# fchchen/omni-recall-rag

Measured on AMD Instinct MI355X. Metric: queries/sec at top-k=10 over N x 3072-d chunks; score delta vs C# reference in `parity`, higher is better.
Workload: dtype i8 screen + f32*f32->f64 exact re-score; 1 GPU; C3: 10000000 chunks x 3072-d fp32 on one GPU, batch=256 queries per step, top-k=10, full hybrid (cosine+keyword+recency), candidate_limit=corpus; corpus_rows=10000000

## Files before the change

include/omnirecall_hip.h:

```cpp
#ifndef OMNIRECALL_HIP_H
#define OMNIRECALL_HIP_H

#include <stddef.h>
#include <stdint.h>

#ifdef __cplusplus
extern "C" {
#endif

#define ORR_ABI_VERSION 1

typedef enum orr_status {
    ORR_OK      = 0,
    ORR_EINVAL  = -1,
    ORR_ENOMEM  = -2,
    ORR_EDEVICE = -3,
    ORR_ECOMM   = -4,
    ORR_EDIM    = -5,
    ORR_ESTATE  = -6
} orr_status;

typedef struct orr_index orr_index;

typedef struct orr_config {
// ... 160 lines not shown
                              int64_t now_ticks, int32_t topk, int64_t candidate_limit, const orr_scope *scope,
                              int64_t *out_rows, double *out_scores, int32_t *out_counts);

int orr_search_batch_in_scopes(orr_index *idx, int32_t B, int32_t dim, const float *q,
                               const uint8_t *terms_utf8, const uint32_t *term_off, const uint32_t *query_term_off,
                               int64_t now_ticks, int32_t topk, int64_t candidate_limit,
                               int32_t n_scopes, const orr_scope *const *scopes, const int32_t *query_scope ,
                               int64_t *out_rows, double *out_scores, int32_t *out_counts);

int orr_index_set_option(orr_index *idx, const char *name, int64_t value);

int orr_index_screen_dots(orr_index *idx, int32_t B, int32_t dim, const float *q, float *out);

int orr_index_screen_i8_dots(orr_index *idx, int32_t B, int32_t dim, const float *q, int32_t form, int32_t nt_rows,
                             int32_t *out_dots, int8_t *out_iq, int8_t *out_ie);

int orr_index_screen_i8_consts(orr_index *idx, int32_t B, int32_t dim, const float *q, float *out_scale, float *out_rel_err,
                               float *out_rel_hat, float *out_rowf, float *out_s1, double *out_err2, double *out_err2_level1,
                               int8_t *out_iq2);

int orr_index_screen_i8_stream_dots(orr_index *idx, int32_t B, int32_t dim, const float *q, int32_t unit16, int32_t *out_dots);

int orr_index_pass_dots(orr_index *idx, int32_t kernel, int32_t B, int32_t dim, const float *q, float *out);

int orr_index_set_profiling(orr_index *idx, int32_t enabled);
int orr_index_kernel_stats(orr_index *idx, orr_kernel_stat *out, int32_t cap);

int orr_index_search_stats(orr_index *idx, orr_search_stats *out, int32_t reset);

typedef struct orr_cluster orr_cluster;
int        orr_cluster_create(const int32_t *devices, int32_t n_shards, int32_t dim, int64_t capacity_rows_per_shard,
                              orr_cluster **out);
void       orr_cluster_destroy(orr_cluster *c);
int32_t    orr_cluster_shards(const orr_cluster *c);
orr_index *orr_cluster_shard(orr_cluster *c, int32_t i);
int        orr_cluster_seal(orr_cluster *c);
int64_t    orr_cluster_rows(const orr_cluster *c);
int        orr_cluster_search_batch(orr_cluster *c, int32_t B, int32_t dim, const float *q_host,
                                    const uint8_t *terms_utf8, const uint32_t *term_off,
                                    const uint32_t *query_term_off, int64_t now_ticks, int32_t topk,
                                    int64_t candidate_limit, int64_t *out_rows, double *out_scores,
                                    int32_t *out_counts);
int        orr_cluster_search_batch_scoped(orr_cluster *c, int32_t B, int32_t dim, const float *q_host,
                                           const uint8_t *terms_utf8, const uint32_t *term_off,
                                           const uint32_t *query_term_off, int64_t now_ticks, int32_t topk,
                                           int64_t candidate_limit, int64_t n_scope_ids, const int64_t *scope_ids,
// ... 20 lines not shown
```

omni-recall-rag_amd/_native.py:

```python
from __future__ import annotations

import ctypes as C
import os

_PKG = os.path.dirname(os.path.abspath(__file__))
HIP_LIB_PATH = os.environ.get("ORR_HIP_LIB") or os.path.join(_PKG, "libomnirecall_hip.so")
HOST_LIB_PATH = os.path.join(_PKG, "libomnirecall_host.so")


class OrrError(RuntimeError):
    def __init__(self, code: int, message: str):
        super().__init__(f"libomnirecall_hip status {code}: {message}")
        self.code = code


ORR_OK, ORR_EINVAL, ORR_ENOMEM, ORR_EDEVICE, ORR_ECOMM, ORR_EDIM, ORR_ESTATE = 0, -1, -2, -3, -4, -5, -6
ORR_CAND_TRAILER, ORR_CAND_DOT_EXACT, ORR_CAND_DEAD = 1, 2, 16
ORR_SCOPE_AND, ORR_SCOPE_OR, ORR_SCOPE_ANDNOT = 0, 1, 2


class OrrConfig(C.Structure):
    _fields_ = [("struct_size", C.c_int32), ("device", C.c_int32), ("dim", C.c_int32), ("flags", C.c_int32),
                ("capacity_rows", C.c_int64), ("row_base", C.c_int64)]

# ... 96 lines not shown
hip.orr_index_update_rows.argtypes = [_vp, _i64, _vp, _i32, _vp, _vp]
hip.orr_index_insert_rows.restype = C.c_int
hip.orr_index_insert_rows.argtypes = [_vp, _i64, _i32, _vp, _vp, _vp, _vp, _vp, _vp]
hip.orr_cluster_insert_rows.restype = C.c_int
hip.orr_cluster_insert_rows.argtypes = [_vp, _i32, _i64, _i32, _vp, _vp, _vp, _vp, _vp, _vp]
hip.orr_index_compact.restype = C.c_int
hip.orr_index_compact.argtypes = [_vp, _vp]
hip.orr_cluster_compact.restype = C.c_int
hip.orr_cluster_compact.argtypes = [_vp, _vp]
hip.orr_index_live_rows.restype = _i64
hip.orr_index_live_rows.argtypes = [_vp]
hip.orr_index_view.restype = C.c_int
hip.orr_index_view.argtypes = [_vp, C.POINTER(_vp)]
hip.orr_index_screen_dots.restype = C.c_int
hip.orr_index_screen_dots.argtypes = [_vp, _i32, _i32, _vp, _vp]
hip.orr_index_screen_i8_dots.restype = C.c_int
hip.orr_index_screen_i8_dots.argtypes = [_vp, _i32, _i32, _vp, _i32, _i32, _vp, _vp, _vp]
hip.orr_index_screen_i8_consts.restype = C.c_int
hip.orr_index_screen_i8_consts.argtypes = [_vp, _i32, _i32, _vp, _vp, _vp, _vp, _vp, _vp, _vp, _vp, _vp]
hip.orr_index_screen_i8_stream_dots.restype = C.c_int
hip.orr_index_screen_i8_stream_dots.argtypes = [_vp, _i32, _i32, _vp, _i32, _vp]
hip.orr_index_pass_dots.restype = C.c_int
hip.orr_index_pass_dots.argtypes = [_vp, _i32, _i32, _i32, _vp, _vp]
hip.orr_index_set_profiling.restype = C.c_int
hip.orr_index_set_profiling.argtypes = [_vp, _i32]
hip.orr_index_kernel_stats.restype = C.c_int
hip.orr_index_kernel_stats.argtypes = [_vp, _vp, _i32]
hip.orr_index_search_stats.restype = C.c_int
hip.orr_index_search_stats.argtypes = [_vp, C.POINTER(OrrSearchStats), _i32]
hip.orr_cluster_create.restype = C.c_int
hip.orr_cluster_create.argtypes = [_vp, _i32, _i32, _i64, C.POINTER(_vp)]
hip.orr_cluster_destroy.restype = None
hip.orr_cluster_destroy.argtypes = [_vp]
hip.orr_cluster_shards.restype = _i32
hip.orr_cluster_shards.argtypes = [_vp]
hip.orr_cluster_shard.restype = _vp
hip.orr_cluster_shard.argtypes = [_vp, _i32]
hip.orr_cluster_seal.restype = C.c_int
hip.orr_cluster_seal.argtypes = [_vp]
hip.orr_cluster_rows.restype = _i64
hip.orr_cluster_rows.argtypes = [_vp]
hip.orr_cluster_search_batch.restype = C.c_int
hip.orr_cluster_search_batch.argtypes = [_vp, _i32, _i32, _vp, _vp, _vp, _vp, _i64, _i32, _i64, _vp, _vp, _vp]
hip.orr_cluster_search_batch_scoped.restype = C.c_int
hip.orr_cluster_search_batch_scoped.argtypes = [_vp, _i32, _i32, _vp, _vp, _vp, _vp, _i64, _i32, _i64, _i64, _vp, _vp, _vp, _vp, _vp]
hip.orr_cluster_search_batch_masked.restype = C.c_int
# ... 61 lines not shown
host.orrh_batcher_create.restype = _vp
host.orrh_batcher_create.argtypes = [_vp, _i32, _i32]
host.orrh_batcher_destroy.restype = None
host.orrh_batcher_destroy.argtypes = [_vp]
host.orrh_batcher_search.restype = C.c_int
host.orrh_batcher_search.argtypes = [_vp, _i32, _vp, _vp, _vp, _i32, _i64, _i32, _i64, _vp, _vp, _vp]
host.orrh_batcher_search_at.restype = C.c_int
host.orrh_batcher_search_at.argtypes = [_vp, _i32, _vp, _vp, _vp, _i32, _i64, _i32, _i64, _vp, _vp, _vp, _vp]
host.orrh_batcher_stats.restype = None
host.orrh_batcher_stats.argtypes = [_vp, _vp, _vp, _vp]
host.orrh_batcher_create.restype = _vp
host.orrh_batcher_create.argtypes = [_vp, _i32, _i32]
host.orrh_batcher_destroy.restype = None
host.orrh_batcher_destroy.argtypes = [_vp]
host.orrh_batcher_search.restype = C.c_int
host.orrh_batcher_search.argtypes = [_vp, _i32, _vp, _vp, _vp, _i32, _i64, _i32, _i64, _vp, _vp, _vp]
host.orrh_batcher_stats.restype = None
host.orrh_batcher_stats.argtypes = [_vp, _vp, _vp, _vp]

EXPORTED_HIP_SYMBOLS = [
    "orr_abi_version", "orr_device_count", "orr_last_error", "orr_index_create", "orr_index_destroy",
    "orr_index_append", "orr_index_seal", "orr_index_rows", "orr_index_dim", "orr_search_batch",
    "orr_search_shard", "orr_search_shard_ex", "orr_search_batch_scoped", "orr_search_batch_masked", "orr_search_batch_masked_groups", "orr_search_shard_scoped", "orr_search_shard_masked", "orr_index_scope_count", "orr_merge_candidates", "orr_merge_candidates_ex", "orr_index_set_profiling", "orr_index_kernel_stats",
    "orr_index_save", "orr_index_load", "orr_index_set_row_base", "orr_index_set_option", "orr_index_screen_dots", "orr_index_screen_i8_dots", "orr_index_screen_i8_consts", "orr_index_screen_i8_stream_dots", "orr_index_pass_dots", "orr_index_view",
    "orr_index_delete_rows", "orr_index_update_rows", "orr_index_insert_rows", "orr_cluster_insert_rows", "orr_index_live_rows", "orr_index_compact", "orr_cluster_compact", "orr_index_search_stats",
    "orr_cluster_create", "orr_cluster_destroy", "orr_cluster_shards", "orr_cluster_shard", "orr_cluster_seal", "orr_cluster_rows",
    "orr_cluster_search_batch", "orr_cluster_search_batch_scoped", "orr_cluster_search_batch_masked", "orr_cluster_search_stats", "orr_cluster_set_option",
    "orr_scope_create", "orr_scope_create_ticks", "orr_scope_add_ids", "orr_scope_combine", "orr_scope_rows", "orr_scope_row_ids", "orr_scope_destroy",
    "orr_search_batch_in_scope", "orr_search_batch_in_scopes",
]
EXPORTED_HOST_SYMBOLS = ["orrh_is_blank", "orrh_lower_invariant", "orrh_query_terms", "orrh_build_snippet",
                         "orrh_round4", "orrh_has_sufficient_evidence", "orrh_format_score_f4", "orrh_last_error", "orrh_store_create", "orrh_store_destroy",
                         "orrh_store_upsert_document", "orrh_store_upsert_chunks", "orrh_store_delete_document",
                         "orrh_store_chunk_count", "orrh_store_import_cosmos_json", "orrh_store_export_cosmos_json", "orrh_service_create", "orrh_service_destroy",
                         "orrh_service_search_json", "orrh_service_search_documents_json", "orrh_service_stats", "orrh_service_tombstoned_rows", "orrh_service_compactions", "orrh_service_delta_merges", "orrh_service_updated_rows", "orrh_service_inserted_rows", "orrh_service_set_option", "orrh_free", "orrh_batcher_create", "orrh_batcher_destroy",
                         "orrh_batcher_search", "orrh_batcher_search_at", "orrh_batcher_stats"]


def check(status: int) -> None:
    if status != ORR_OK:
        raise OrrError(status, (hip.orr_last_error() or b"").decode("utf-8", "replace"))
```

omni-recall-rag_amd/csrc/orr_api.hip:

```cpp
#include <hip/hip_runtime.h>

#include <algorithm>
#include <cmath>
#include <cstdarg>
#include <cstdio>
#include <chrono>
#include <pthread.h>
#include <dlfcn.h>
#include <atomic>
#include <condition_variable>
#include <functional>
#include <cstring>
#include <limits>
#include <mutex>
#include <shared_mutex>
#include <deque>
#include <new>
#include <numeric>
#include <string>
#include <string_view>
#include <thread>
#include <unordered_map>
#include <vector>

// ... 3209 lines not shown
                HIP_TRY(orr::launch_fuse_select(io.d_dot, io.d_dotf, n, idx->d_norm_b, idx->d_created, io.d_rowc, io.kw, qc, a.now_ticks,
                                                n, B, 0, sample_seg, nullptr, idx->ws_sel.as<orr::SelEntry>(), 0, s));
            }
            Timed t(idx, "select_floor", 0.0);
            HIP_TRY(orr::launch_select_final_sample(idx->ws_sel.as<orr::SelEntry>(), n_seg32, sample_seg, B, kprime, d_tau, s));
        }
        {
            Timed t(idx, "fuse_select", (double)B * (double)n * (8.0 * (p.use_cos ? 1 : 0) + 8.0 + 8.0));
            HIP_TRY(orr::launch_fuse_select(io.d_dot, io.d_dotf, n, idx->d_norm_b, idx->d_created, io.d_rowc, io.kw, qc, a.now_ticks,
                                            n, B, sample_seg, n_seg32 - sample_seg, d_tau, idx->ws_sel.as<orr::SelEntry>(), 0, s));
        }
        Timed t(idx, "select_final", (double)B * (double)n_seg * orr::kSelWidth * sizeof(orr::SelEntry));
        HIP_TRY(orr::launch_select_final(idx->ws_sel.as<orr::SelEntry>(), n_seg32, B, kprime, n, idx->row_base,
                                         io.d_dot, io.d_dotf, n, idx->d_norm_b, idx->d_created, idx->d_row_ids, io.kw,
                                         p.use_mfma ? 0 : 1, p.approx_eps, nullptr, nullptr, 0u, nullptr, io.d_cand, s));
    }
    if (p.use_mfma && !p.two_stage()) {
        Timed t(idx, "rescore_exact", (double)B * kprime * 4.0 * idx->dim);
        HIP_TRY(orr::launch_rescore_exact(idx->d_emb, idx->dim, io.d_q, B, kprime, idx->row_base, io.d_cand, s));
    }
    return ORR_OK;
}

int finish_pass(orr_index *idx, const BatchArgs &a, const PassPlan &p, const KwSide &kws, uint32_t n_terms_total)
{
    const int32_t B = a.B;
    HIP_TRY(hipStreamSynchronize(idx->stream));
    if (kws.bm_bytes) {
        if (kws.bm_bytes >= ((size_t)16 << 20)) {
            HIP_TRY(hipMemsetAsync(idx->ws_bitmaps.p, 0, kws.bm_bytes, idx->stream_aux));
            HIP_TRY(hipEventRecord(idx->ev_bm_clean, idx->stream_aux));
            idx->bm_clean_pending = true;
        } else {
            HIP_TRY(hipMemsetAsync(idx->ws_bitmaps.p, 0, kws.bm_bytes, idx->stream_kw));
        }
        idx->bitmaps_clean = std::max(kws.bm_bytes, kws.bm_clean_before);
    }
    if (n_terms_total > 0 && idx->ws_counter.p) {
        HIP_TRY(hipMemsetAsync(idx->ws_counter.p, 0, sizeof(unsigned long long), idx->stream_kw));
        if (idx->ws_kwalias.p) HIP_TRY(hipMemsetAsync(idx->ws_kwalias.p, 0, idx->ws_kwalias.cap, idx->stream_kw));
        idx->kw_counters_clean = true;
        idx->kw_counters_of[0] = idx->ws_counter.p;
        idx->kw_counters_of[1] = idx->ws_kwalias.p;
    }
    if (p.dev_norms) memcpy(idx->h_norm_a.data(), idx->pin_norm.p, sizeof(double) * (size_t)B);
    if (n_terms_total > 0) {
        idx->sstats.kw_hits_total += (int64_t)(*idx->pin_kwcnt.as<unsigned long long>() >> 32);
        idx->sstats.kw_passes += 1;
    }
    if (p.two_stage()) {
        idx->h_survivors.assign(idx->pin_cnt.as<uint32_t>(), idx->pin_cnt.as<uint32_t>() + B);
        uint64_t sum = 0;
        for (uint32_t cnt : idx->h_survivors) sum += cnt;
        const uint64_t mean = p.masked ? 1024 : sum / (uint64_t)B;
        if (mean > 4096 && idx->sample_boost < 16) idx->sample_boost *= 2;
        else if (mean < 512 && idx->sample_boost > 1) idx->sample_boost /= 2;
    }
    g_ht.mark(4);
    collect_events(idx);
    if (kws.overflow_possible) {
        const unsigned long long cnt = *idx->pin_kwcnt.as<unsigned long long>();
        const uint32_t hits = (uint32_t)(cnt >> 32);
        if (hits > kws.max_hits) {
            if ((uint64_t)hits * sizeof(orr::KwHit) > ((uint64_t)8 << 30))
                return fail(ORR_ENOMEM, "keyword terms matched %u vocabulary tokens: a hit list of that size is refused (8 GiB)", hits);
            idx->kw_hits_cap = hits + hits / 4 + 1024u;
            return kRetryPass;
        }
    }
    return ORR_OK;
}

int run_shard_once(orr_index *idx, const BatchArgs &a, int32_t kprime, bool host_records, const float **q_host,
                   const orr_candidate **recs_host, PassPlan &p)
{
    g_ht.start();
    ORR_TRY(bind_device(idx));
    const int64_t n = participating_rows(idx, a.candidate_limit);
    const int32_t B = a.B;
    hipStream_t s = idx->stream;
    if (recs_host) *recs_host = nullptr;

    PassFront f;
    ORR_TRY(open_pass(idx, a, kprime, [&](const std::vector<uint32_t> &qoff, PassPlan &plan) { return plan_pass(idx, a, kprime, n, qoff, plan); },
                      host_records, true, true, q_host, p, f));
    PassIo &io = f.io;

    if (p.form == PassForm::Empty) {
        const std::vector<orr_candidate> empty = empty_records(B, kprime);
        if (io.direct_host) memcpy(io.d_cand, empty.data(), f.rec_bytes);
        else HIP_TRY(hipMemcpyAsync(io.d_cand, empty.data(), f.rec_bytes, hipMemcpyHostToDevice, s));
        HIP_TRY(hipStreamSynchronize(s));
        if (f.q_download_pending || p.dev_norms) HIP_TRY(hipEventSynchronize(idx->ev_q));
        if (recs_host && io.direct_host) *recs_host = io.d_cand;
        return ORR_OK;
    }

    if (p.screen == Screen::GemvI8) ORR_TRY(launch_i8_query_image(idx, io.d_q, B, false, s));

    KwSide kws;
    ORR_TRY(launch_keyword_side(idx, a, f.qoff, kws));
    io.kw = kws.view;
    g_ht.mark(1);

    ORR_TRY(launch_numerators(idx, a, p, n, io));
    g_ht.mark(0);

    ORR_TRY(launch_consts(idx, a, p, n, f.qoff, f.q_download_pending, io));
    if (f.n_terms_total > 0) HIP_TRY(hipStreamWaitEvent(s, idx->ev_kw_done, 0));
    g_ht.mark(2);

    ORR_TRY(launch_selection(idx, a, p, kprime, n, io, host_records, f.rec_bytes));

    if (!owner_of(idx)->dead.empty())
        HIP_TRY(orr::launch_mark_dead_records(io.d_cand, B, kprime, owner_of(idx)->d_dead.as<int64_t>(),
                                              (int32_t)owner_of(idx)->dead.size(), idx->row_base, s));
    if (host_records) ORR_TRY(records_to_host(idx, f, s));
    g_ht.mark(3);
    idx->sstats.pass_mode = p.pass_mode();

    const int r = finish_pass(idx, a, p, kws, f.n_terms_total);
    if (r != ORR_OK) return r;
    if (recs_host && io.direct_host) *recs_host = io.d_cand;
    else if (recs_host && host_records) *recs_host = idx->pin_cand.as<orr_candidate>();
    return ORR_OK;
}

template <class Pass>
int retry_pass(orr_index *idx, Pass &&once)
{
    for (int attempt = 0;; ++attempt) {
// ... 1325 lines not shown

extern "C" {

int orr_index_search_stats(orr_index *idx, orr_search_stats *out, int32_t reset)
{
    if (!idx) return fail(ORR_EINVAL, "orr_index_search_stats: null index");
    LanePool::Exclusive all(pool_of(idx));
    std::lock_guard<std::mutex> lock(idx->mu);
    idx->sstats.survivor_capacity = idx->survivor_cap;
    idx->sstats.vocab_tokens = idx->n_tokens;
    if (out) {
        *out = idx->sstats;
        for_each_lane(idx, [&](orr_index *l) {
            if (l == idx) return;
            l->sstats.survivor_capacity = l->survivor_cap;
            escalation::add_search_stats(*out, l->sstats);
        });
    }
    if (reset) {
        auto clear = [](orr_index *x) { const int64_t cap = x->survivor_cap; x->sstats = orr_search_stats{}; x->sstats.survivor_capacity = cap; };
        for_each_lane(idx, clear);
    }
    return ORR_OK;
}

static int shard_pass_into(orr_index *idx, BatchArgs a, int32_t kprime, int64_t candidate_limit, orr_candidate *out, size_t first,
                           bool dev_out)
{
    const int32_t B = a.B;
    const size_t rec_q = sizeof(orr_candidate) * ((size_t)kprime + 1);
    unsigned char *dst = reinterpret_cast<unsigned char *>(out) + rec_q * first;
    a.out_dev = dev_out ? reinterpret_cast<orr_candidate *>(dst) : nullptr;
    PassPlan pass;
    ORR_TRY(run_shard(idx, a, kprime, false, nullptr, nullptr, pass));
    if (!dev_out) HIP_TRY(hipMemcpy(dst, idx->ws_cand.p, rec_q * (size_t)B, hipMemcpyDefault));
    idx->sstats.passes += 1;
    const int64_t n = participating_rows(idx, candidate_limit);
    std::vector<int32_t> active((size_t)B);
    std::iota(active.begin(), active.end(), 0);
    for (int round = 0; round < 4; ++round) {
        const ShardOutcome kept = outcome_of(idx, pass, n);
        if (!kept.kept(active.size())) break;
        escalation::account_survivors(idx->sstats, kept, active.size());
        std::vector<int32_t> over;
        uint32_t worst = 0, cap = 0;
        for (size_t i = 0; i < active.size(); ++i)
// ... 1098 lines not shown
```

omni-recall-rag_amd/csrc/orr_gemm.hip:

```cpp
#include "orr_kernels.h"
#include "orr_device.h"
#include "orr_epilogue.h"

#include <algorithm>
#include <cstdio>
#include <vector>
#include <cstdlib>

namespace orr {

typedef float f32x4v __attribute__((ext_vector_type(4)));

constexpr int kGemmBK = 64;


constexpr int kBfLd = 72;

__device__ __forceinline__ void split_write(__bf16 *hi_img, __bf16 *lo_img, int r, int c4, const float4 &v)
{
    const __bf16 h0 = (__bf16)v.x, h1 = (__bf16)v.y, h2 = (__bf16)v.z, h3 = (__bf16)v.w;
    bf16x4 h, l;
    h[0] = h0; h[1] = h1; h[2] = h2; h[3] = h3;
    l[0] = (__bf16)(v.x - (float)h0);
    l[1] = (__bf16)(v.y - (float)h1);
    l[2] = (__bf16)(v.z - (float)h2);
// ... 150 lines not shown
            __builtin_amdgcn_sched_barrier(0);
            __syncthreads();
            mfma_step();
        }
    }
    if (!FUSED) {
#pragma unroll
        for (int i = 0; i < 2; ++i)
#pragma unroll
            for (int j = 0; j < NT; ++j) {
                const int64_t col = n0 + wn * 32 * NT + j * 32 + fr;
#pragma unroll
                for (int e = 0; e < 16; ++e) {
                    const int row = b0 + wm * 64 + i * 32 + (e & 3) + 8 * (e >> 2) + 4 * fh;
                    if (row < B && col < n_rows) S[(int64_t)row * s_stride + col] = acc[i][j][e];
                }
            }
    } else {
        __syncthreads();
        fused_epilogue<2, NT, PROD == 1>(acc, b0 + wm * 64, n0 + wn * 32 * NT, B, n_rows, epi, lane, reinterpret_cast<EpiParked *>(img) + tid, 512);
    }
}

template <int BITS>
__global__ __launch_bounds__(256) void query_count_planes_kernel(KwView kw, int32_t B, int64_t n_rows, int64_t plane_stride,
                                                                uint32_t *__restrict__ planes, int64_t oct_first, int64_t oct_end)
{
    constexpr int kCountPlanes = BITS;
    const int g = blockIdx.y;
    const int32_t n_qg = gridDim.y;
    const int lane = threadIdx.x & 63, q = lane & 31, h = lane >> 5;
    const int b = g * 32 + q;
    uint32_t t0 = 0, t1 = 0;
    if (b < B) { t0 = kw.q_term_off[b]; t1 = kw.q_term_off[b + 1]; }
    const bool saturate = BITS == 4 && t1 - t0 > 15u;
    const int64_t n_quads = kw.words_per_term >> 2;
    const int64_t wave_id = ((int64_t)blockIdx.x * blockDim.x + threadIdx.x) >> 6, n_waves = ((int64_t)gridDim.x * blockDim.x) >> 6;
    for (int64_t pr = oct_first + wave_id; pr < oct_end; pr += n_waves) {
        const int64_t Q = pr * 2 + h;
        uint32_t c[4][kCountPlanes];
#pragma unroll
        for (int k = 0; k < 4; ++k)
#pragma unroll
            for (int p = 0; p < kCountPlanes; ++p) c[k][p] = 0u;
        if (Q < n_quads) {
            for (uint32_t i = t0; i < t1; ++i) {
                const uint4 w4 = *reinterpret_cast<const uint4 *>(kw.bitmaps + kw_term_base(kw, kw.q_term_idx[i]) + Q * 4);
                const uint32_t wv[4] = {w4.x, w4.y, w4.z, w4.w};
#pragma unroll
                for (int k = 0; k < 4; ++k) {
                    uint32_t carry = wv[k];
                    if (saturate) { c[k][0] |= carry; continue; }
#pragma unroll
                    for (int p = 0; p < kCountPlanes; ++p) {
                        const uint32_t t = c[k][p] & carry;
                        c[k][p] ^= carry;
                        carry = t;
                    }
                }
            }
            if (saturate) {
#pragma unroll
                for (int k = 0; k < 4; ++k)
#pragma unroll
                    for (int p = 1; p < kCountPlanes; ++p) c[k][p] = c[k][0];
            }
        }
#pragma unroll
        for (int k = 0; k < 4; ++k) {
#pragma unroll
            for (int p = 0; p < kCountPlanes; ++p) {
                uint32_t x = c[k][p];
#pragma unroll
                for (int s = 4; s >= 0; --s) {
                    const int jj = 1 << s;
                    const uint32_t low = s == 4 ? 0x0000FFFFu : s == 3 ? 0x00FF00FFu : s == 2 ? 0x0F0F0F0Fu : s == 1 ? 0x33333333u : 0x55555555u;
                    const uint32_t y = (uint32_t)__shfl_xor((int)x, jj, 64);
                    x = (q & jj) ? (((y & ~low) >> jj) | (x & ~low)) : ((x & low) | ((y & low) << jj));
                }
                c[k][p] = x;
            }
            const int64_t row = (Q * 4 + k) * 32 + q;
            if (BITS == 2) {
                if (row < n_rows) {
#pragma unroll
                    for (int kk = 0; kk < 2; ++kk) {
                        uint32_t wv = 0u;
#pragma unroll
                        for (int p = 0; p < 2; ++p) {
                            uint32_t x = (c[k][p] >> (16 * kk)) & 0xFFFFu;
                            x = (x | (x << 8)) & 0x00FF00FFu;
                            x = (x | (x << 4)) & 0x0F0F0F0Fu;
                            x = (x | (x << 2)) & 0x33333333u;
                            x = (x | (x << 1)) & 0x55555555u;
                            wv |= x << p;
                        }
                        planes[((int64_t)kk * n_qg + g) * plane_stride + row] = wv;
                    }
                }
            } else if (row < n_rows) {
#pragma unroll
                for (int kk = 0; kk < 4; ++kk) {
                    uint32_t wv = 0u;
#pragma unroll
                    for (int p = 0; p < kCountPlanes; ++p) {
                        uint32_t x = (c[k][p] >> (8 * kk)) & 0xFFu;
                        x = (x | (x << 12)) & 0x000F000Fu;
                        x = (x | (x << 6)) & 0x03030303u;
                        x = (x | (x << 3)) & 0x11111111u;
                        wv |= x << p;
                    }
                    planes[((int64_t)kk * n_qg + g) * plane_stride + row] = wv;
                }
            }
        }
    }
}

hipError_t launch_query_count_planes(KwView kw, int32_t B, int64_t n_rows, int64_t plane_stride, uint32_t *planes, hipStream_t s,
                                     int64_t row_first, int64_t row_end, int32_t bits)
{
    if (B <= 0 || !kw.bitmaps || n_rows <= 0) return hipSuccess;
    if (kw.words_per_term % 4 != 0 || row_first % 256 != 0) return hipErrorInvalidValue;
    const int64_t n_oct = (kw.words_per_term / 4 + 1) / 2;
    const int64_t oct_first = row_first / 256;
    const int64_t oct_end = row_end < 0 ? n_oct : std::min<int64_t>(n_oct, (row_end + 255) / 256);
    if (oct_end <= oct_first) return hipSuccess;
    int64_t bx = (oct_end - oct_first + 3) / 4;
    if (bx > 2048) bx = 2048;
    if (bits == 2)
        hipLaunchKernelGGL(query_count_planes_kernel<2>, dim3((unsigned)bx, (unsigned)((B + 31) / 32)), dim3(256), 0, s, kw, B, n_rows,
                           plane_stride, planes, oct_first, oct_end);
    else
        hipLaunchKernelGGL(query_count_planes_kernel<4>, dim3((unsigned)bx, (unsigned)((B + 31) / 32)), dim3(256), 0, s, kw, B, n_rows,
                           plane_stride, planes, oct_first, oct_end);
    return hipGetLastError();
}

__device__ __forceinline__ float4 fused_query_const_of(const QueryConst &c, unsigned long long tau_b, const float *i8_qs1, const double *i8_qerr2, int b)
{
    float4 o;
    o.x = c.use_cos ? (float)(c.inv_sqrt_na * 0.7) : 0.f;
    if (tau_b <= 1ull) {
        o.y = -__builtin_huge_valf();
    } else {
        const double floor_score = key_score(tau_b);
        const double margin = 1e-5 * (1.0 + fabs(floor_score));
        o.y = __double2float_rd(floor_score - margin);
    }
    o.z = c.n_terms > 0 ? __double2float_ru(0.2 / (double)(c.n_terms > 15 ? 15 : c.n_terms)) : 0.f;
    o.w = 0.f;
    if (i8_qs1) {
        o.x *= i8_qs1[b];
        o.w = c.use_cos ? __double2float_ru(0.7 * 1.000001 * sqrt(i8_qerr2[b]) * c.inv_sqrt_na) : 0.f;
    }
    return o;
}

// ... 983 lines not shown
```

omni-recall-rag_amd/index.py:

```python
from __future__ import annotations

import ctypes as C
from typing import List, Optional, Sequence, Tuple

import numpy as np

from . import _native as N

CAND_DTYPE = np.dtype([("approx_score", "<f8"), ("dot", "<f8"), ("norm_b", "<f8"), ("created_ticks", "<i8"),
                       ("row_id", "<i8"), ("order_key", "<i8"), ("matches", "<i4"), ("flags", "<i4")])
assert CAND_DTYPE.itemsize == C.sizeof(N.OrrCandidate) == 56


def _is_torch(x) -> bool:
    return type(x).__module__.startswith("torch")


def _ptr(x) -> Optional[int]:
    if x is None:
        return None
    if _is_torch(x):
        assert x.is_contiguous()
        if x.is_cuda:
            import torch
# ... 427 lines not shown
        if qvecs is not None:
            q = np.ascontiguousarray(qvecs, dtype=np.float32)
            q = q.reshape(1, -1) if q.ndim == 1 else q
            B, dim = int(q.shape[0]), int(q.shape[1])
            out.update(s1=np.empty(B, np.float32), err2=np.empty(B, np.float64), err2_level1=np.empty(B, np.float64),
                       iq2=np.empty((B, dim), np.int8))
        N.check(N.hip.orr_index_screen_i8_consts(self._h, B, dim, _ptr(q), _ptr(out["scale"]), _ptr(out["rel_err"]), _ptr(out["rel_hat"]),
                                                 _ptr(out["rowf"]), _ptr(out.get("s1")), _ptr(out.get("err2")),
                                                 _ptr(out.get("err2_level1")), _ptr(out.get("iq2"))))
        return out

    def screen_i8_stream_dots(self, qvecs, unit16: bool = False) -> np.ndarray:
        q = np.ascontiguousarray(qvecs, dtype=np.float32)
        q = q.reshape(1, -1) if q.ndim == 1 else q
        out = np.empty((q.shape[0], 2, self.rows), dtype=np.int32)
        N.check(N.hip.orr_index_screen_i8_stream_dots(self._h, int(q.shape[0]), int(q.shape[1]), _ptr(q), 1 if unit16 else 0, _ptr(out)))
        return out

    def pass_dots(self, qvecs, kernel: int) -> np.ndarray:
        q = np.ascontiguousarray(qvecs, dtype=np.float32)
        q = q.reshape(1, -1) if q.ndim == 1 else q
        out = np.empty((q.shape[0], self.rows), dtype=np.float32)
        N.check(N.hip.orr_index_pass_dots(self._h, int(kernel), int(q.shape[0]), int(q.shape[1]), _ptr(q), _ptr(out)))
        return out

    def set_profiling(self, on) -> None:
        N.check(N.hip.orr_index_set_profiling(self._h, int(on)))

    def search_stats(self, reset: bool = False) -> dict:
        st = N.OrrSearchStats()
        N.check(N.hip.orr_index_search_stats(self._h, C.byref(st), 1 if reset else 0))
        d = {n: int(getattr(st, n)) for n, _ in N.OrrSearchStats._fields_ if n != "reserved"}
        d["survivors_per_query"] = d["survivors_total"] / d["survivor_samples"] if d["survivor_samples"] else None
        return d

    def reset_search_stats(self) -> None:
        N.check(N.hip.orr_index_search_stats(self._h, None, 1))

    def kernel_stats(self) -> dict:
        cap = 64
        while True:
            arr = (N.OrrKernelStat * cap)()
            n = N.hip.orr_index_kernel_stats(self._h, C.cast(arr, C.c_void_p), cap)
            if n <= cap:
                break
            cap = n
# ... 198 lines not shown
```

Measured before the change: 30930 queries/s.

## Restructure keyword count-plane kernel with shared-memory transpose and reorder pass launches

Rewrites the keyword count-plane kernel so each wave reads a run of bitmap words per query word group. It transposes the 32x32 bit block in registers via a shared helper, stages the result in shared memory, and writes coalesced uint4 stores with a z-grid dimension over count words. The shard pass now launches the numerators, and the query constants when they are computed on device, before the keyword side, so they can overlap. It also adds a count_words API and a host selftest, and splits finish_pass into helpers. The aim is to cut the cost of the bit-sliced keyword counting and its shuffle-heavy transpose, at the price of more shared memory and a larger grid.

```diff
diff --git a/include/omnirecall_hip.h b/include/omnirecall_hip.h
--- a/include/omnirecall_hip.h
+++ b/include/omnirecall_hip.h
@@ -206,6 +206,9 @@
 int orr_index_screen_i8_stream_dots(orr_index *idx, int32_t B, int32_t dim, const float *q, int32_t unit16, int32_t *out_dots);
 
 int orr_index_pass_dots(orr_index *idx, int32_t kernel, int32_t B, int32_t dim, const float *q, float *out);
+
+int orr_index_count_words(orr_index *idx, int32_t B, const uint8_t *terms_utf8, const uint32_t *term_off, const uint32_t *query_term_off,
+                          int32_t bits, int64_t row_first, int64_t row_end, uint32_t *out);
 
 int orr_index_set_profiling(orr_index *idx, int32_t enabled);
 int orr_index_kernel_stats(orr_index *idx, orr_kernel_stat *out, int32_t cap);
diff --git a/omni-recall-rag_amd/_native.py b/omni-recall-rag_amd/_native.py
--- a/omni-recall-rag_amd/_native.py
+++ b/omni-recall-rag_amd/_native.py
@@ -142,6 +142,8 @@
 hip.orr_index_screen_i8_stream_dots.argtypes = [_vp, _i32, _i32, _vp, _i32, _vp]
 hip.orr_index_pass_dots.restype = C.c_int
 hip.orr_index_pass_dots.argtypes = [_vp, _i32, _i32, _i32, _vp, _vp]
+hip.orr_index_count_words.restype = C.c_int
+hip.orr_index_count_words.argtypes = [_vp, _i32, _vp, _vp, _vp, _i32, _i64, _i64, _vp]
 hip.orr_index_set_profiling.restype = C.c_int
 hip.orr_index_set_profiling.argtypes = [_vp, _i32]
 hip.orr_index_kernel_stats.restype = C.c_int
@@ -249,7 +251,7 @@
     "orr_abi_version", "orr_device_count", "orr_last_error", "orr_index_create", "orr_index_destroy",
     "orr_index_append", "orr_index_seal", "orr_index_rows", "orr_index_dim", "orr_search_batch",
     "orr_search_shard", "orr_search_shard_ex", "orr_search_batch_scoped", "orr_search_batch_masked", "orr_search_batch_masked_groups", "orr_search_shard_scoped", "orr_search_shard_masked", "orr_index_scope_count", "orr_merge_candidates", "orr_merge_candidates_ex", "orr_index_set_profiling", "orr_index_kernel_stats",
-    "orr_index_save", "orr_index_load", "orr_index_set_row_base", "orr_index_set_option", "orr_index_screen_dots", "orr_index_screen_i8_dots", "orr_index_screen_i8_consts", "orr_index_screen_i8_stream_dots", "orr_index_pass_dots", "orr_index_view",
+    "orr_index_save", "orr_index_load", "orr_index_set_row_base", "orr_index_set_option", "orr_index_screen_dots", "orr_index_screen_i8_dots", "orr_index_screen_i8_consts", "orr_index_screen_i8_stream_dots", "orr_index_pass_dots", "orr_index_count_words", "orr_index_view",
     "orr_index_delete_rows", "orr_index_update_rows", "orr_index_insert_rows", "orr_cluster_insert_rows", "orr_index_live_rows", "orr_index_compact", "orr_cluster_compact", "orr_index_search_stats",
     "orr_cluster_create", "orr_cluster_destroy", "orr_cluster_shards", "orr_cluster_shard", "orr_cluster_seal", "orr_cluster_rows",
     "orr_cluster_search_batch", "orr_cluster_search_batch_scoped", "orr_cluster_search_batch_masked", "orr_cluster_search_stats", "orr_cluster_set_option",
diff --git a/omni-recall-rag_amd/csrc/host/orr_count_words_selftest.cpp b/omni-recall-rag_amd/csrc/host/orr_count_words_selftest.cpp
--- /dev/null
+++ b/omni-recall-rag_amd/csrc/host/orr_count_words_selftest.cpp
@@ -0,0 +1,165 @@
+#include <algorithm>
+#include <cstdio>
+#include <cstdlib>
+#include <random>
+#include <vector>
+
+#include "../orr_count_words.h"
+
+static int g_failed = 0;
+#define CHECK(cond)                                                                  \
+    do {                                                                             \
+        if (!(cond)) { printf("FAILED %s:%d: %s\n", __FILE__, __LINE__, #cond); ++g_failed; } \
+    } while (0)
+
+namespace cw = count_words;
+
+struct Group {
+    std::vector<uint32_t> term_word;
+    std::vector<std::vector<int>> q_terms;
+};
+
+template <int BITS>
+static void words_by_rules(const Group &g, int kk, uint32_t *a)
+{
+    for (int n = 0; n < cw::queries_per_word(BITS); ++n) {
+        uint32_t *c = a + cw::column_of(BITS, n, 0);
+        for (int p = 0; p < BITS; ++p) c[p] = 0u;
+        const size_t q = (size_t)(kk * cw::queries_per_word(BITS) + n);
+        if (q >= g.q_terms.size()) continue;
+        const bool sat = cw::saturate(BITS, (uint32_t)g.q_terms[q].size());
+        for (int t : g.q_terms[q]) {
+            if (sat) cw::saturate_or(c, g.term_word[(size_t)t]);
+            else cw::ripple_add<BITS>(c, g.term_word[(size_t)t]);
+        }
+        if (sat) cw::saturate_fill<BITS>(c);
+    }
+    cw::transpose32(a);
+}
+
+static uint32_t naive_count(const Group &g, size_t q, int row, int bits)
+{
+    if (q >= g.q_terms.size()) return 0u;
+    uint32_t cnt = 0;
+    for (int t : g.q_terms[q]) cnt += (g.term_word[(size_t)t] >> row) & 1u;
+    if (bits == 4 && g.q_terms[q].size() > 15) return cnt ? 15u : 0u;
+    return cnt;
+}
+
+template <int BITS>
+static void check_group(const Group &g, int rows_valid = 32)
+{
+    for (int kk = 0; kk < cw::words_per_group(BITS); ++kk) {
+        uint32_t a[32];
+        words_by_rules<BITS>(g, kk, a);
+        for (int row = 0; row < rows_valid; ++row) {
+            uint32_t want = 0;
+            for (int n = 0; n < cw::queries_per_word(BITS); ++n)
+                want |= naive_count(g, (size_t)(kk * cw::queries_per_word(BITS) + n), row, BITS) << (BITS * n);
+            if (a[row] != want) { CHECK(!"a count word differs from the pair-by-pair count"); return; }
+        }
+    }
+}
+
+static void test_transpose()
+{
+    std::mt19937 rng(1);
+    for (int rep = 0; rep < 200; ++rep) {
+        uint32_t a[32], b[32];
+        for (auto &v : a) v = rep == 0 ? 0u : rep == 1 ? 0xFFFFFFFFu : rng();
+        if (rep == 2) for (int i = 0; i < 32; ++i) a[i] = 1u << i;
+        if (rep == 3) for (int i = 0; i < 32; ++i) a[i] = i == 5 ? 0x80000001u : 0u;
+        std::copy(a, a + 32, b);
+        cw::transpose32(b);
+        bool same = true;
+        for (int i = 0; i < 32; ++i)
+            for (int j = 0; j < 32; ++j) same = same && (((b[i] >> j) & 1u) == ((a[j] >> i) & 1u));
+        CHECK(same);
+        cw::transpose32(b);
+        CHECK(std::equal(a, a + 32, b));
+    }
+}
+
+static void test_rules()
+{
+    CHECK(cw::words_per_group(2) == 2 && cw::words_per_group(4) == 4 && cw::queries_per_word(2) == 16 && cw::queries_per_word(4) == 8);
+    CHECK(!cw::saturate(4, 15) && cw::saturate(4, 16) && cw::saturate(4, 65535) && !cw::saturate(2, 16));
+    for (int bits : {2, 4})
+        for (int n = 0; n < 32 / bits; ++n)
+            for (int p = 0; p < bits; ++p) CHECK(cw::column_of(bits, n, p) == bits * n + p);
+    uint32_t c[4] = {0, 0, 0, 0};
+    for (int i = 1; i <= 16; ++i) {
+        cw::ripple_add<4>(c, 0x0000FFFFu);
+        for (int p = 0; p < 4; ++p) CHECK(c[p] == ((((uint32_t)i & 15u) >> p) & 1u ? 0x0000FFFFu : 0u));
+    }
+}
+
+template <int BITS>
+static void test_every_value_everywhere()
+{
+    const int max_v = BITS == 2 ? 3 : 15;
+    for (int q = 0; q < 32; ++q)
+        for (int v = 0; v <= max_v; ++v)
+            for (int row : {0, 1, 15, 16, 30, 31}) {
+                Group g;
+                g.q_terms.resize(32);
+                for (int i = 0; i < v; ++i) { g.q_terms[(size_t)q].push_back((int)g.term_word.size()); g.term_word.push_back(1u << row); }
+                if (v < max_v) { g.q_terms[(size_t)q].push_back((int)g.term_word.size()); g.term_word.push_back(~(1u << row)); }
+                check_group<BITS>(g);
+            }
+}
+
+static void test_saturation()
+{
+    std::mt19937 rng(9);
+    for (int q : {0, 7, 8, 31})
+        for (int n_terms : {16, 17, 40}) {
+            Group g;
+            g.q_terms.resize(32);
+            for (int i = 0; i < n_terms; ++i) { g.q_terms[(size_t)q].push_back(i); g.term_word.push_back(rng() & rng() & rng()); }
+            g.term_word[0] |= 1u;
+            for (auto &w : g.term_word) w &= ~2u;
+            for (auto &w : g.term_word) w |= 4u;
+            g.q_terms[(size_t)(q ^ 1)] = {0, 1, 2};
+            check_group<4>(g);
+        }
+    Group g;
+    g.q_terms.resize(32);
+    for (int i = 0; i < 15; ++i) { g.q_terms[3].push_back(i); g.term_word.push_back(i == 0 ? 0xFFFFFFFFu : 0x0000FFFFu); }
+    check_group<4>(g);
+}
+
+template <int BITS>
+static void test_random()
+{
+    std::mt19937 rng(BITS);
+    for (int rep = 0; rep < 300; ++rep) {
+        Group g;
+        const int n_q = rep % 5 == 0 ? 1 + (int)(rng() % 32) : 32;
+        const int n_t = 1 + (int)(rng() % 60);
+        for (int t = 0; t < n_t; ++t) g.term_word.push_back(rep % 3 == 0 ? rng() & rng() : rng());
+        g.q_terms.resize((size_t)n_q);
+        for (auto &qt : g.q_terms) {
+            const int k = BITS == 2 ? (int)(rng() % 4) : (rng() % 9 == 0 ? 16 + (int)(rng() % 30) : (int)(rng() % 16));
+            for (int i = 0; i < k; ++i) qt.push_back((int)(rng() % (uint32_t)n_t));
+        }
+        const int rows_valid = rep % 4 == 0 ? 1 + (int)(rng() % 31) : 32;
+        if (rows_valid < 32)
+            for (auto &w : g.term_word) w &= (1u << rows_valid) - 1u;
+        check_group<BITS>(g, rows_valid);
+    }
+}
+
+int main()
+{
+    test_transpose();
+    test_rules();
+    test_every_value_everywhere<2>();
+    test_every_value_everywhere<4>();
+    test_saturation();
+    test_random<2>();
+    test_random<4>();
+    if (g_failed) { printf("orr_count_words_selftest: %d check(s) FAILED\n", g_failed); return 1; }
+    printf("orr_count_words_selftest: ok\n");
+    return 0;
+}
diff --git a/omni-recall-rag_amd/csrc/orr_api.hip b/omni-recall-rag_amd/csrc/orr_api.hip
--- a/omni-recall-rag_amd/csrc/orr_api.hip
+++ b/omni-recall-rag_amd/csrc/orr_api.hip
@@ -3255,10 +3255,8 @@
     return ORR_OK;
 }
 
-int finish_pass(orr_index *idx, const BatchArgs &a, const PassPlan &p, const KwSide &kws, uint32_t n_terms_total)
-{
-    const int32_t B = a.B;
-    HIP_TRY(hipStreamSynchronize(idx->stream));
+int clear_keyword_side(orr_index *idx, const KwSide &kws, uint32_t n_terms_total)
+{
     if (kws.bm_bytes) {
         if (kws.bm_bytes >= ((size_t)16 << 20)) {
             HIP_TRY(hipMemsetAsync(idx->ws_bitmaps.p, 0, kws.bm_bytes, idx->stream_aux));
@@ -3276,11 +3274,31 @@
         idx->kw_counters_of[0] = idx->ws_counter.p;
         idx->kw_counters_of[1] = idx->ws_kwalias.p;
     }
-    if (p.dev_norms) memcpy(idx->h_norm_a.data(), idx->pin_norm.p, sizeof(double) * (size_t)B);
     if (n_terms_total > 0) {
         idx->sstats.kw_hits_total += (int64_t)(*idx->pin_kwcnt.as<unsigned long long>() >> 32);
         idx->sstats.kw_passes += 1;
     }
+    return ORR_OK;
+}
+
+int keyword_hits_overflowed(orr_index *idx, const KwSide &kws)
+{
+    if (!kws.overflow_possible) return ORR_OK;
+    const unsigned long long cnt = *idx->pin_kwcnt.as<unsigned long long>();
+    const uint32_t hits = (uint32_t)(cnt >> 32);
+    if (hits <= kws.max_hits) return ORR_OK;
+    if ((uint64_t)hits * sizeof(orr::KwHit) > ((uint64_t)8 << 30))
+        return fail(ORR_ENOMEM, "keyword terms matched %u vocabulary tokens: a hit list of that size is refused (8 GiB)", hits);
+    idx->kw_hits_cap = hits + hits / 4 + 1024u;
+    return kRetryPass;
+}
+
+int finish_pass(orr_index *idx, const BatchArgs &a, const PassPlan &p, const KwSide &kws, uint32_t n_terms_total)
+{
+    const int32_t B = a.B;
+    HIP_TRY(hipStreamSynchronize(idx->stream));
+    ORR_TRY(clear_keyword_side(idx, kws, n_terms_total));
+    if (p.dev_norms) memcpy(idx->h_norm_a.data(), idx->pin_norm.p, sizeof(double) * (size_t)B);
     if (p.two_stage()) {
         idx->h_survivors.assign(idx->pin_cnt.as<uint32_t>(), idx->pin_cnt.as<uint32_t>() + B);
         uint64_t sum = 0;
@@ -3291,17 +3309,7 @@
     }
     g_ht.mark(4);
     collect_events(idx);
-    if (kws.overflow_possible) {
-        const unsigned long long cnt = *idx->pin_kwcnt.as<unsigned long long>();
-        const uint32_t hits = (uint32_t)(cnt >> 32);
-        if (hits > kws.max_hits) {
-            if ((uint64_t)hits * sizeof(orr::KwHit) > ((uint64_t)8 << 30))
-                return fail(ORR_ENOMEM, "keyword terms matched %u vocabulary tokens: a hit list of that size is refused (8 GiB)", hits);
-            idx->kw_hits_cap = hits + hits / 4 + 1024u;
-            return kRetryPass;
-        }
-    }
-    return ORR_OK;
+    return keyword_hits_overflowed(idx, kws);
 }
 
 int run_shard_once(orr_index *idx, const BatchArgs &a, int32_t kprime, bool host_records, const float **q_host,
@@ -3330,16 +3338,20 @@
     }
 
     if (p.screen == Screen::GemvI8) ORR_TRY(launch_i8_query_image(idx, io.d_q, B, false, s));
+    ORR_TRY(launch_numerators(idx, a, p, n, io));
+    g_ht.mark(0);
+    const bool consts_first = p.dev_norms && !f.q_download_pending;
+    if (consts_first) {
+        ORR_TRY(launch_consts(idx, a, p, n, f.qoff, f.q_download_pending, io));
+        g_ht.mark(2);
+    }
 
     KwSide kws;
     ORR_TRY(launch_keyword_side(idx, a, f.qoff, kws));
     io.kw = kws.view;
     g_ht.mark(1);
 
-    ORR_TRY(launch_numerators(idx, a, p, n, io));
-    g_ht.mark(0);
-
-    ORR_TRY(launch_consts(idx, a, p, n, f.qoff, f.q_download_pending, io));
+    if (!consts_first) ORR_TRY(launch_consts(idx, a, p, n, f.qoff, f.q_download_pending, io));
     if (f.n_terms_total > 0) HIP_TRY(hipStreamWaitEvent(s, idx->ev_kw_done, 0));
     g_ht.mark(2);
 
@@ -4711,6 +4723,50 @@
         for_each_lane(idx, clear);
     }
     return ORR_OK;
+}
+
+int orr_index_count_words(orr_index *idx, int32_t B, const uint8_t *terms_utf8, const uint32_t *term_off, const uint32_t *query_term_off,
+                          int32_t bits, int64_t row_first, int64_t row_end, uint32_t *out)
+{
+    const char *fn = "orr_index_count_words";
+    if (!idx || !query_term_off || !out || B <= 0) return fail(ORR_EINVAL, "%s: bad argument", fn);
+    if (bits != 2 && bits != 4) return fail(ORR_EINVAL, "%s: bits must be 2 or 4", fn);
+    if (row_first < 0 || row_first % 256 != 0) return fail(ORR_EINVAL, "%s: row_first must be a non-negative multiple of 256", fn);
+    std::vector<uint32_t> qoff(query_term_off, query_term_off + (size_t)B + 1);
+    for (int32_t b = 0; b < B; ++b) {
+        if (qoff[b + 1] < qoff[b]) return fail(ORR_EINVAL, "%s: query_term_off is not monotone at query %d", fn, b);
+        if (qoff[b + 1] - qoff[b] > 65535) return fail(ORR_EINVAL, "%s: query %d has more than 65535 terms", fn, b);
+        if (bits == 2 && qoff[b + 1] - qoff[b] > 3) return fail(ORR_EINVAL, "%s: two-bit words hold at most three terms (query %d)", fn, b);
+    }
+    const uint32_t n_terms_total = qoff[(size_t)B] - qoff[0];
+    if (n_terms_total > 0 && (!term_off || !terms_utf8)) return fail(ORR_EINVAL, "%s: terms are referenced but term_off/terms_utf8 is NULL", fn);
+    LanePool::Exclusive all(pool_of(idx));
+    std::lock_guard<std::mutex> lock(idx->mu);
+    if (!idx->sealed) return fail(ORR_ESTATE, "%s: the index is not sealed", fn);
+    const int64_t n = idx->n_rows;
+    if (n <= 0) return ORR_OK;
+    ORR_TRY(bind_device(idx));
+    BatchArgs a{};
+    a.B = B; a.terms_utf8 = terms_utf8; a.term_off = term_off; a.query_term_off = query_term_off;
+    const int64_t plane_stride = (n + 63) / 64 * 64;
+    const size_t n_words = (size_t)bits * (size_t)((B + 31) / 32);
+    return retry_pass(idx, [&]() -> int {
+        hipStream_t k = idx->stream_kw;
+        KwSide kws;
+        ORR_TRY(launch_keyword_side(idx, a, qoff, kws));
+        ORR_TRY(idx->ws_fany.reserve(sizeof(uint32_t) * orr::kCountPlanes * (size_t)((B + 31) / 32) * (size_t)plane_stride));
+        HIP_TRY(hipMemsetAsync(idx->ws_fany.p, 0xAB, sizeof(uint32_t) * n_words * (size_t)plane_stride, k));
+        {
+            Timed t(idx, "count_planes", (bits == 2 ? 8.0 : 16.0) * (double)((B + 31) / 32) * (double)((row_end < 0 ? n : std::min(row_end, n)) - std::min(row_first, n)), k);
+            HIP_TRY(orr::launch_query_count_planes(kws.view, B, n, plane_stride, idx->ws_fany.as<uint32_t>(), k, row_first, row_end, bits));
+        }
+        HIP_TRY(hipMemcpy2DAsync(out, sizeof(uint32_t) * (size_t)n, idx->ws_fany.p, sizeof(uint32_t) * (size_t)plane_stride,
+                                 sizeof(uint32_t) * (size_t)n, n_words, hipMemcpyDefault, k));
+        HIP_TRY(hipStreamSynchronize(k));
+        ORR_TRY(clear_keyword_side(idx, kws, n_terms_total));
+        collect_events(idx);
+        return keyword_hits_overflowed(idx, kws);
+    });
 }
 
 static int shard_pass_into(orr_index *idx, BatchArgs a, int32_t kprime, int64_t candidate_limit, orr_candidate *out, size_t first,
diff --git a/omni-recall-rag_amd/csrc/orr_count_words.h b/omni-recall-rag_amd/csrc/orr_count_words.h
--- /dev/null
+++ b/omni-recall-rag_amd/csrc/orr_count_words.h
@@ -0,0 +1,60 @@
+#pragma once
+
+#include <cstdint>
+
+#if defined(__HIPCC__)
+#define ORR_CW_HD __host__ __device__ __forceinline__
+#define ORR_CW_UNROLL _Pragma("unroll")
+#else
+#define ORR_CW_HD inline
+#define ORR_CW_UNROLL
+#endif
+
+namespace count_words {
+
+constexpr int kGroupQueries = 32;
+constexpr int words_per_group(int bits) { return bits; }
+constexpr int queries_per_word(int bits) { return 32 / bits; }
+constexpr uint32_t kMaxCount4 = 15u;
+
+ORR_CW_HD bool saturate(int bits, uint32_t n_terms) { return bits == 4 && n_terms > kMaxCount4; }
+
+ORR_CW_HD constexpr int column_of(int bits, int n, int p) { return bits * n + p; }
+
+template <int BITS>
+ORR_CW_HD void ripple_add(uint32_t *c, uint32_t w)
+{
+    uint32_t carry = w;
+ORR_CW_UNROLL
+    for (int p = 0; p < BITS; ++p) {
+        const uint32_t t = c[p] & carry;
+        c[p] ^= carry;
+        carry = t;
+    }
+}
+
+ORR_CW_HD void saturate_or(uint32_t *c, uint32_t w) { c[0] |= w; }
+template <int BITS>
+ORR_CW_HD void saturate_fill(uint32_t *c)
+{
+ORR_CW_UNROLL
+    for (int p = 1; p < BITS; ++p) c[p] = c[0];
+}
+
+ORR_CW_HD void transpose32(uint32_t *a)
+{
+ORR_CW_UNROLL
+    for (int s = 4; s >= 0; --s) {
+        const int j = 1 << s;
+        const uint32_t m = s == 4 ? 0x0000FFFFu : s == 3 ? 0x00FF00FFu : s == 2 ? 0x0F0F0F0Fu : s == 1 ? 0x33333333u : 0x55555555u;
+ORR_CW_UNROLL
+        for (int k = 0; k < 32; ++k) {
+            if (k & j) continue;
+            const uint32_t t = ((a[k] >> j) ^ a[k + j]) & m;
+            a[k + j] ^= t;
+            a[k] ^= t << j;
+        }
+    }
+}
+
+}
diff --git a/omni-recall-rag_amd/csrc/orr_gemm.hip b/omni-recall-rag_amd/csrc/orr_gemm.hip
--- a/omni-recall-rag_amd/csrc/orr_gemm.hip
+++ b/omni-recall-rag_amd/csrc/orr_gemm.hip
@@ -1,6 +1,7 @@
 #include "orr_kernels.h"
 #include "orr_device.h"
 #include "orr_epilogue.h"
+#include "orr_count_words.h"
 
 #include <algorithm>
 #include <cstdio>
@@ -197,97 +198,83 @@
     }
 }
 
+template <int BITS, bool OFFS>
+__device__ __forceinline__ void count_word_columns(const KwView &kw, int32_t B, int b0, const uint32_t *__restrict__ bm, int lane, uint32_t *a)
+{
+    namespace cw = count_words;
+    constexpr int kSlots = BITS == 2 ? 3 : 4;
+    auto word_of = [&](uint32_t i, bool on) {
+        const uint32_t t = kw.q_term_idx[i];
+        const int64_t base = OFFS ? kw.term_word_off[t] : (int64_t)t * kw.words_per_term;
+        return (bm + base)[lane] & (on ? 0xFFFFFFFFu : 0u);
+    };
+#pragma unroll
+    for (int n = 0; n < cw::queries_per_word(BITS); ++n) {
+        uint32_t *c = a + cw::column_of(BITS, n, 0);
+#pragma unroll
+        for (int p = 0; p < BITS; ++p) c[p] = 0u;
+        const int b = b0 + n < B ? b0 + n : B - 1;
+        const uint32_t t0 = kw.q_term_off[b], t1 = t0 + ((kw.q_term_off[b + 1] - t0) & (b0 + n < B ? 0xFFFFFFFFu : 0u));
+        if (BITS == 2) {
+            uint32_t w[kSlots];
+#pragma unroll
+            for (int j = 0; j < kSlots; ++j) w[j] = word_of(t0 + j < t1 ? t0 + j : 0u, t0 + j < t1);
+#pragma unroll
+            for (int j = 0; j < kSlots; ++j) cw::ripple_add<BITS>(c, w[j]);
+        } else {
+            const bool sat = cw::saturate(BITS, t1 - t0);
+            for (uint32_t i = t0; i < t1; i += kSlots) {
+                uint32_t w[kSlots];
+#pragma unroll
+                for (int j = 0; j < kSlots; ++j) w[j] = word_of(i + j < t1 ? i + j : i, i + j < t1);
+#pragma unroll
+                for (int j = 0; j < kSlots; ++j) {
+                    if (sat) cw::saturate_or(c, w[j]);
+                    else cw::ripple_add<BITS>(c, w[j]);
+                }
+            }
+            if (sat) cw::saturate_fill<BITS>(c);
+        }
+    }
+}
+
+constexpr int kCountRunWords = 64;
+constexpr int kCountStagePitch = 9;
+
 template <int BITS>
-__global__ __launch_bounds__(256) void query_count_planes_kernel(KwView kw, int32_t B, int64_t n_rows, int64_t plane_stride,
-                                                                uint32_t *__restrict__ planes, int64_t oct_first, int64_t oct_end)
-{
-    constexpr int kCountPlanes = BITS;
-    const int g = blockIdx.y;
+__global__ __launch_bounds__(256) void query_count_planes_kernel(KwView kw, int32_t B, int64_t row_lim, int64_t plane_stride,
+                                                                uint32_t *__restrict__ planes, int64_t word_first, int64_t word_end)
+{
+    __shared__ uint4 stage[4][kCountRunWords * kCountStagePitch];
+    const int g = blockIdx.y, kk = blockIdx.z;
     const int32_t n_qg = gridDim.y;
-    const int lane = threadIdx.x & 63, q = lane & 31, h = lane >> 5;
-    const int b = g * 32 + q;
-    uint32_t t0 = 0, t1 = 0;
-    if (b < B) { t0 = kw.q_term_off[b]; t1 = kw.q_term_off[b + 1]; }
-    const bool saturate = BITS == 4 && t1 - t0 > 15u;
-    const int64_t n_quads = kw.words_per_term >> 2;
-    const int64_t wave_id = ((int64_t)blockIdx.x * blockDim.x + threadIdx.x) >> 6, n_waves = ((int64_t)gridDim.x * blockDim.x) >> 6;
-    for (int64_t pr = oct_first + wave_id; pr < oct_end; pr += n_waves) {
-        const int64_t Q = pr * 2 + h;
-        uint32_t c[4][kCountPlanes];
-#pragma unroll
-        for (int k = 0; k < 4; ++k)
-#pragma unroll
-            for (int p = 0; p < kCountPlanes; ++p) c[k][p] = 0u;
-        if (Q < n_quads) {
-            for (uint32_t i = t0; i < t1; ++i) {
-                const uint4 w4 = *reinterpret_cast<const uint4 *>(kw.bitmaps + kw_term_base(kw, kw.q_term_idx[i]) + Q * 4);
-                const uint32_t wv[4] = {w4.x, w4.y, w4.z, w4.w};
-#pragma unroll
-                for (int k = 0; k < 4; ++k) {
-                    uint32_t carry = wv[k];
-                    if (saturate) { c[k][0] |= carry; continue; }
-#pragma unroll
-                    for (int p = 0; p < kCountPlanes; ++p) {
-                        const uint32_t t = c[k][p] & carry;
-                        c[k][p] ^= carry;
-                        carry = t;
-                    }
-                }
-            }
-            if (saturate) {
-#pragma unroll
-                for (int k = 0; k < 4; ++k)
-#pragma unroll
-                    for (int p = 1; p < kCountPlanes; ++p) c[k][p] = c[k][0];
-            }
-        }
-#pragma unroll
-        for (int k = 0; k < 4; ++k) {
-#pragma unroll
-            for (int p = 0; p < kCountPlanes; ++p) {
-                uint32_t x = c[k][p];
-#pragma unroll
-                for (int s = 4; s >= 0; --s) {
-                    const int jj = 1 << s;
-                    const uint32_t low = s == 4 ? 0x0000FFFFu : s == 3 ? 0x00FF00FFu : s == 2 ? 0x0F0F0F0Fu : s == 1 ? 0x33333333u : 0x55555555u;
-                    const uint32_t y = (uint32_t)__shfl_xor((int)x, jj, 64);
-                    x = (q & jj) ? (((y & ~low) >> jj) | (x & ~low)) : ((x & low) | ((y & low) << jj));
-                }
-                c[k][p] = x;
-            }
-            const int64_t row = (Q * 4 + k) * 32 + q;
-            if (BITS == 2) {
-                if (row < n_rows) {
-#pragma unroll
-                    for (int kk = 0; kk < 2; ++kk) {
-                        uint32_t wv = 0u;
-#pragma unroll
-                        for (int p = 0; p < 2; ++p) {
-                            uint32_t x = (c[k][p] >> (16 * kk)) & 0xFFFFu;
-                            x = (x | (x << 8)) & 0x00FF00FFu;
-                            x = (x | (x << 4)) & 0x0F0F0F0Fu;
-                            x = (x | (x << 2)) & 0x33333333u;
-                            x = (x | (x << 1)) & 0x55555555u;
-                            wv |= x << p;
-                        }
-                        planes[((int64_t)kk * n_qg + g) * plane_stride + row] = wv;
-                    }
-                }
-            } else if (row < n_rows) {
-#pragma unroll
-                for (int kk = 0; kk < 4; ++kk) {
-                    uint32_t wv = 0u;
-#pragma unroll
-                    for (int p = 0; p < kCountPlanes; ++p) {
-                        uint32_t x = (c[k][p] >> (8 * kk)) & 0xFFu;
-                        x = (x | (x << 12)) & 0x000F000Fu;
-                        x = (x | (x << 6)) & 0x03030303u;
-                        x = (x | (x << 3)) & 0x11111111u;
-                        wv |= x << p;
-                    }
-                    planes[((int64_t)kk * n_qg + g) * plane_stride + row] = wv;
-                }
-            }
+    const int lane = threadIdx.x & 63, wave = threadIdx.x >> 6;
+    const int64_t W0 = word_first + ((int64_t)blockIdx.x * 4 + wave) * kCountRunWords;
+    const int64_t W0r = W0 < word_end ? W0 : word_first;
+    const int ln = W0r + lane < word_end ? lane : 0;
+    const uint32_t *__restrict__ bm = kw.bitmaps + W0r;
+    uint32_t a[32];
+    const int b0 = g * count_words::kGroupQueries + kk * count_words::queries_per_word(BITS);
+    if (kw.term_word_off) count_word_columns<BITS, true>(kw, B, b0, bm, ln, a);
+    else count_word_columns<BITS, false>(kw, B, b0, bm, ln, a);
+    count_words::transpose32(a);
+    uint4 *st = stage[wave];
+#pragma unroll
+    for (int i = 0; i < 8; ++i) st[lane * kCountStagePitch + i] = make_uint4(a[4 * i], a[4 * i + 1], a[4 * i + 2], a[4 * i + 3]);
+    __syncthreads();
+    uint32_t *__restrict__ out = planes + ((int64_t)kk * n_qg + g) * plane_stride;
+#pragma unroll
+    for (int j = 0; j < 8; ++j) {
+        const int qd = j * 64 + lane;
+        const uint4 v = st[(qd >> 3) * kCountStagePitch + (qd & 7)];
+        const int64_t row = W0 * 32 + (int64_t)qd * 4;
+        if (row + 3 < row_lim) {
+            *reinterpret_cast<uint4 *>(out + row) = v;
+        } else {
+            const uint32_t e[4] = {v.x, v.y, v.z, v.w};
+#pragma unroll
+            for (int r = 0; r < 4; ++r)
+                if (row + r < row_lim) out[row + r] = e[r];
         }
     }
 }
@@ -296,19 +283,19 @@
                                      int64_t row_first, int64_t row_end, int32_t bits)
 {
     if (B <= 0 || !kw.bitmaps || n_rows <= 0) return hipSuccess;
-    if (kw.words_per_term % 4 != 0 || row_first % 256 != 0) return hipErrorInvalidValue;
+    if (kw.words_per_term % 4 != 0 || row_first % 256 != 0 || plane_stride % 4 != 0) return hipErrorInvalidValue;
     const int64_t n_oct = (kw.words_per_term / 4 + 1) / 2;
     const int64_t oct_first = row_first / 256;
     const int64_t oct_end = row_end < 0 ? n_oct : std::min<int64_t>(n_oct, (row_end + 255) / 256);
     if (oct_end <= oct_first) return hipSuccess;
-    int64_t bx = (oct_end - oct_first + 3) / 4;
-    if (bx > 2048) bx = 2048;
+    const int64_t word_first = oct_first * 8, word_end = std::min<int64_t>(oct_end * 8, kw.words_per_term);
+    const int64_t row_lim = std::min<int64_t>(n_rows, word_end * 32);
+    const int64_t bx = (word_end - word_first + 4 * kCountRunWords - 1) / (4 * kCountRunWords);
+    const dim3 grid((unsigned)bx, (unsigned)((B + 31) / 32), (unsigned)count_words::words_per_group(bits == 2 ? 2 : 4));
     if (bits == 2)
-        hipLaunchKernelGGL(query_count_planes_kernel<2>, dim3((unsigned)bx, (unsigned)((B + 31) / 32)), dim3(256), 0, s, kw, B, n_rows,
-                           plane_stride, planes, oct_first, oct_end);
+        hipLaunchKernelGGL(query_count_planes_kernel<2>, grid, dim3(256), 0, s, kw, B, row_lim, plane_stride, planes, word_first, word_end);
     else
-        hipLaunchKernelGGL(query_count_planes_kernel<4>, dim3((unsigned)bx, (unsigned)((B + 31) / 32)), dim3(256), 0, s, kw, B, n_rows,
-                           plane_stride, planes, oct_first, oct_end);
+        hipLaunchKernelGGL(query_count_planes_kernel<4>, grid, dim3(256), 0, s, kw, B, row_lim, plane_stride, planes, word_first, word_end);
     return hipGetLastError();
 }
 
diff --git a/omni-recall-rag_amd/index.py b/omni-recall-rag_amd/index.py
--- a/omni-recall-rag_amd/index.py
+++ b/omni-recall-rag_amd/index.py
@@ -473,6 +473,13 @@
         q = q.reshape(1, -1) if q.ndim == 1 else q
         out = np.empty((q.shape[0], self.rows), dtype=np.float32)
         N.check(N.hip.orr_index_pass_dots(self._h, int(kernel), int(q.shape[0]), int(q.shape[1]), _ptr(q), _ptr(out)))
+        return out
+
+    def count_words(self, queries_terms, bits: int = 4, row_first: int = 0, row_end: int = -1) -> np.ndarray:
+        pool, toff, qoff = pack_terms(queries_terms)
+        B = int(qoff.shape[0]) - 1
+        out = np.empty((int(bits), (B + 31) // 32, self.rows), dtype=np.uint32)
+        N.check(N.hip.orr_index_count_words(self._h, B, _ptr(pool), _ptr(toff), _ptr(qoff), int(bits), int(row_first), int(row_end), _ptr(out)))
         return out
 
     def set_profiling(self, on) -> None:
```

After: 31360 queries/s, median of 6. 1.4% higher.
